# tonyckc/WT-PSE-code

Hardware: AMD Instinct MI355X
Metric: training images/sec (256x256 fundus) — full WT-PSE iteration (higher is better)
Workload: dtype f32 (layers with > 16 output channels and the fused 1x1 heads: x2h (2 fp16 terms per fp32 operand — power-of-two operand scaling —, 3 fp16 MFMA products per multiply, fp32 accumulation); the 16-channel layers the same on 16x16x32, the 1-/3-channel input layers and small 1x1 convs fp32-input MFMA)

## Files before the change

include/wtpse_hip.h:

```cpp
#ifndef WTPSE_HIP_H
#define WTPSE_HIP_H
#ifdef __cplusplus
extern "C" {
#endif


int wtpse_pack_conv_weights(const float* params, const int* desc, int n_desc, float* packed, void* stream);

int wtpse_conv_fwd(const float* in0, int C0, const float* in1, int C1, const float* wpacked, const float* bias,
                   const float* pro0, const float* pro1, int pro_relu, float* out0, float* out1, int Csplit, float* stats,
                   int B, int H, int W, int Cout, int ksize, int relu_out, const float* mask_ref, unsigned* out_amax, void* stream);
int wtpse_conv_stats_blocks(int B, int H, int W);
int wtpse_conv_fwd_gram(const float* in0, int C0, const float* wpacked, const float* bias, const float* pro0, int pro_relu,
                        float* out0, float* gram_partial, int B, int H, int W, int Cout, int relu_out, unsigned* out_amax,
                        void* stream);

int wtpse_conv_x3_stats_blocks(int B, int H, int W, int Cout, int ksize);
int wtpse_x3r_enable(int on);
int wtpse_x3_xcd(int on);
int wtpse_x3_small_wide(int on);
int wtpse_x3_terms(int terms);
int wtpse_amax(const float* x, long long n, unsigned* amax_table, void* stream);
int wtpse_pack_conv_weights_x3(const float* params, const int* desc, int n_desc, unsigned short* packed, void* stream);
int wtpse_conv_fwd_x3(const float* in0, int C0, const float* in1, int C1, const unsigned short* wpacked, const float* bias,
                      const float* pro0, const float* pro1, int pro_relu, float* out0, float* out1, int Csplit, float* stats,
                      int B, int H, int W, int Cout, int ksize, int relu_out, const float* mask_ref, const unsigned* in_amax,
                      const unsigned* in_amax1, unsigned* out_amax, void* stream);

int wtpse_conv16_x3(const float* in0, int C0, const unsigned short* wx16, const float* bias, const float* pro0, int pro_relu,
                    float* out0, float* stats, float* gram_partial, const float* mask_ref, const float* bn_ss,
                    const float* bn_mean, int bn_relu, int B, int H, int W, int Cout, int relu_out, int in_is_grad,
                    const unsigned* in_amax, unsigned* out_amax, void* stream);
int wtpse_pack_conv16_x3(const float* params, const int* desc, int n_desc, unsigned short* packed, void* stream);

int wtpse_dgrad_bnb(const float* dy, int C, const float* wpacked, float* out0, float* out1, int Csplit, const float* bn_y,
                    const float* bn_ss, const float* bn_mean, int bn_relu, int bn_c0, int bn_c1, float* stats, int B, int H, int W,
                    int Cout, int ksize, void* stream);
int wtpse_dgrad_x3_bnb(const float* dy, int C, const unsigned short* wpacked, float* out0, float* out1, int Csplit,
                       const float* bn_y, const float* bn_ss, const float* bn_mean, int bn_relu, int bn_c0, int bn_c1, float* stats,
                       int B, int H, int W, int Cout, int ksize, const unsigned* in_amax, void* stream);

int wtpse_conv_fwd_bnf(const float* in0, int C0, const float* in1, int C1, const void* wpacked, int layout, const float* bias,
                       const float* pro0, const float* pro1, int pro_relu, float* out0, float* stats, const float* gamma,
                       const float* beta, float* running_mean, float* running_var, long long* num_batches, float momentum, float eps,
                       float* scale_shift, float* save_mean, float* save_invstd, double* partial2, unsigned* tickets, int B, int H,
// ... 72 lines not shown
                                   int HW, unsigned* amax, void* stream);
int wtpse_bn_bwd_finalize_coef_frozen(const float* stats_partial, int nblk, int C, const float* gamma, const float* invstd,
                                      float* coef, float* dgamma, float* dbeta, float* dbias, int accumulate, void* stream);
int wtpse_bn_bwd_scale_coef(const float* g, const float* coef, float* dy, int B, int C, int HW, unsigned* amax, void* stream);

int wtpse_wt_loss_fwd(const float* z, int B, int C, int HW, float eps, float margin, int domain_num, int per_domain,
                      float* partial, float* gram, float* v, float* offdiag, float* diag, double* rowval,
                      float* dmmd_dv, float* losses, void* stream);
int wtpse_wt_split(int B, int HW, int* chunk_out);
int wtpse_wt_loss_fwd_partials(const float* partial, int S, int B, int HW, float eps, float margin, int domain_num,
                               int per_domain, float* gram, float* v, float* offdiag, float* diag, double* rowval,
                               float* dmmd_dv, float* losses, void* stream);
int wtpse_wt_gram_fwd(const float* z, int B, int C, int HW, float eps, float* partial, float* gram, float* v, float* offdiag,
                      float* diag, void* stream);
int wtpse_wt_final(const float* offdiag, const float* diag, int B, int Bnorm, float margin, const double* rowval, int R,
                   float* losses, void* stream);
int wtpse_wt_loss_bwd(const float* z, int B, int C, int HW, float margin, int domain_num, int per_domain,
                      const float* gram, const float* offdiag, const float* diag, const float* dmmd_dv,
                      const float* g_off, const float* g_diag, const float* g_dom, float w_off, float w_diag, float w_dom,
                      float* Mws, float* dz, int accumulate, void* stream);
int wtpse_wt_combine(const float* losses, int nmaps, float den, int mode, float* out, void* stream);
int wtpse_mmd_fwd(const float* v, int domain_num, int per_domain, double* rowval, float* dmmd_dv, void* stream);

int wtpse_maxpool2_fwd(const float* x, const float* pro, int relu, float* out, int B, int C, int H, int W, void* stream);
int wtpse_maxpool2_bwd(const float* x, const float* pro, int relu, const float* dout, float* dx, int accumulate, int B,
                       int C, int H, int W, void* stream);
int wtpse_maxpool2_bwd_stats_blocks(int B, int H, int W);
int wtpse_maxpool2_bwd_bnb(const float* x, const float* pro, int relu, const float* dout, float* dx, int accumulate,
                           const float* mean, float* stats, int B, int C, int H, int W, void* stream);
int wtpse_upsample2x_fwd(const float* x, const float* pro, int relu, float* out, int B, int C, int H, int W, void* stream);
int wtpse_upsample2x_bwd(const float* dout, float* dx, int accumulate, int B, int C, int H, int W, unsigned* amax, void* stream);
int wtpse_upsample2x_bwd_bn(const float* g, const float* bn_y, const float* bn_coef, float* dx, int B, int C, int H, int W,
                            unsigned* amax, void* stream);
int wtpse_upsample2x_fwd_stats(const float* x, float* out, float* stats, int B, int C, int H, int W, void* stream);
int wtpse_upsample2x_stats_blocks(int B, int H, int W);

int wtpse_resize_bilinear(const float* x, float* out, int B, int C, int H, int W, int Ho, int Wo, void* stream);

int wtpse_attn_fuse_fwd(const float* z, const float* wb, const float* emb, float coef, float* att, float* att_pre,
                        float* mask, float* fuse, int B, int CE, int HW, void* stream);
int wtpse_attn_fuse_bwd(const float* dfuse, const float* z, const float* emb, const float* att, const float* wb, float coef,
                        float* demb, float* dz, float* partial, float* d_wb, int accumulate, int B, int CE, int HW,
                        void* stream);

int wtpse_reparam_fwd(const float* mu, const float* logvar, const float* eps, float* z, long long n, void* stream);
int wtpse_reparam_bwd(const float* dz, const float* logvar, const float* eps, float* dlogvar, long long n, void* stream);
int wtpse_exp_half(const float* logvar, float* std_, long long n, void* stream);
int wtpse_reparam_student(const float* mu, const float* std_, const float* eps, float* z, long long n, void* stream);
int wtpse_nan_scrub(float* x, long long n, int* flag, void* stream);
int wtpse_randn(float* out, long long n, unsigned long long seed, unsigned long long offset,
                const unsigned long long* offset_dev, void* stream);
int wtpse_counter_add(void* counter, long long inc, int is64, void* stream);

int wtpse_reduce_blocks(long long n);
int wtpse_bce_sigmoid_fwd(const float* x, const float* t, long long n, float* partial, float* loss, void* stream);
int wtpse_bce_sigmoid_bwd(const float* x, const float* t, const float* g, float w, long long n, float* dx, void* stream);
int wtpse_pos_weight(const float* mask, const float* t, long long n, float* partial, float* sums, float* pw, void* stream);
int wtpse_pos_weight_from_sums(const float* sums, float* pw, void* stream);
int wtpse_bce_logits_pw_fwd(const float* x, const float* mask, const float* t, const float* pw, long long n, float* partial,
                            float* loss, void* stream);
int wtpse_bce_logits_pw_bwd(const float* x, const float* mask, const float* t, const float* pw, const float* g, float w,
                            long long n, float* dx, void* stream);
int wtpse_mse_fwd(const float* a, const float* b, long long n, float* partial, float* loss, void* stream);
int wtpse_mse_bwd(const float* a, const float* b, const float* g, float w, long long n, float* da, void* stream);
int wtpse_roi(const float* image, const float* logit, float* roi, float* od_pred, int B, int C, int HW, void* stream);
int wtpse_adam(float* p, const float* g, float* m, float* v, long long n, double lr, double beta1, double beta2, double eps,
// ... 118 lines not shown
```

wt-pse-code_amd/wtpse_hip/csrc/conv.hip:

```cpp
#include "internal.h"

#define WTPSE_P16_KC(KS) ((KS) == 3 ? 4 : 8)

struct ConvArgs {
  const float* in0;
  const float* in1;
  const float* wp;
  const float* bias;
  const float* pro0;
  const float* pro1;
  float* out0;
  float* out1;
  float* stats;
  const float* mask;
  const unsigned* in_amax;
  float in_scale;
  unsigned* out_amax;
  float* gram;
  const float* bn_ss;
  const float* bn_mean;
  int bn_c0, bn_c1, bn_relu;
  BnbTail tail;
  BnfTail ftail;
  int B, H, W;
  int C0, C1, Cin, CinP;
  int Cout, CoutP, Csplit;
  int pro_relu;
  int relu_out;
  int tiles_x, tiles_y;
  int xcd_tiles;
};


template <bool P16> struct AccT { typedef f32x16 type; };
template <> struct AccT<true> { typedef f32x4 type; };
__device__ __forceinline__ f32x4 mfma(float a, float b, f32x4 c) { return mfma16(a, b, c); }
__device__ __forceinline__ f32x16 mfma(float a, float b, f32x16 c) { return mfma32(a, b, c); }

template <int PE>
struct PlaneStride {
  static constexpr int value = ((PE - 16 + 31) / 32) * 32 + 16;
};

template <int KS, int MODE, int TWL, bool DB, int EPI>
__global__ __launch_bounds__(256, 3) void conv_fwd_k(ConvArgs a) {
  constexpr bool MASK = EPI == 1, BNB = EPI == 2;
  constexpr int TAPS = KS * KS, PAD = KS / 2;
  constexpr int TW = 1 << TWL, TH = 256 / TW;
  constexpr int PITCH = TW + 2 * PAD, ROWS = TH + 2 * PAD;
  constexpr int PE = PITCH * ROWS;
  constexpr int NPOS = (PE + 255) / 256;
  constexpr int S = PlaneStride<NPOS * 256>::value;
  constexpr bool XP = (MODE == 3 || MODE == 4);
  constexpr int XT = MODE == 4 ? 2 : 3;
  constexpr bool P16 = (MODE == 0) || XP;
  static_assert(!XP || KS == 3, "MODE 3 / 4 is the 3x3 path");
  constexpr int MT = P16 ? 1 : MODE;
  constexpr int MB = P16 ? 16 : 32;
  constexpr int CB = MB * MT;
  constexpr int NT = P16 ? 4 : 2;
  constexpr int NB = P16 ? 16 : 32;
  constexpr int KC = P16 ? WTPSE_P16_KC(KS) : 8;
  constexpr int KQ = P16 ? 4 : 2;
  constexpr int NACC = P16 ? 4 : 16;
  constexpr int CB4 = CB / 4;
  constexpr int NW = (KC * TAPS * CB4 + 255) / 256;
  constexpr int PEP = (PE + 7) & ~7;
  constexpr int XS_SZ = XP ? 2 * XT * PEP * 4 : KC * S;
  constexpr int WS_SZ = XP ? 0 : NW * 1024;
  constexpr int GRAM_SZ = (P16 && KS == 3) ? 4 * 16 * 65 + 4 * 256 : 0;
  constexpr int RED_SZ = 4 * CB * 2 > GRAM_SZ ? 4 * CB * 2 : GRAM_SZ;
  constexpr int MAIN_SZ = (XS_SZ + WS_SZ) > RED_SZ ? (XS_SZ + WS_SZ) : RED_SZ;
  __shared__ __attribute__((aligned(16))) float smem[MAIN_SZ + CB + (BNB ? 4 * CB : 0)];
  float* bias_s = smem + MAIN_SZ;
  const float* bnp_s = bias_s + CB;
  float* Xs = smem;
  float* Ws = smem + XS_SZ;

  const int tid = threadIdx.x, lane = tid & 63, wave = tid >> 6;
  int tile = (int)blockIdx.x, cblk = (int)blockIdx.y;
  if (a.xcd_tiles > 0) {
    const int L = (int)(blockIdx.y * gridDim.x + blockIdx.x), sl = L >> 3;
    cblk = sl % (int)gridDim.y;
    tile = (L & 7) * a.xcd_tiles + sl / (int)gridDim.y;
  }
  int bx = tile;
  const int tx = bx % a.tiles_x;
  bx /= a.tiles_x;
  const int ty = bx % a.tiles_y;
  const int b = bx / a.tiles_y;
  const int cout0 = cblk * CB;
  const int HW = a.H * a.W;
  if (tid < CB) bias_s[tid] = (a.bias && cout0 + tid < a.Cout) ? a.bias[cout0 + tid] : 0.f;
  if (BNB && tid < CB) bnb_stage<CB>(bias_s + CB + tid, cout0 + tid, a);

  int off[NT];
#pragma unroll
  for (int nt = 0; nt < NT; ++nt) {
    int p = wave * 64 + nt * NB + (lane & (NB - 1));
    off[nt] = (p >> TWL) * PITCH + (p & (TW - 1));
  }

  typename AccT<P16>::type acc[MT][NT];
// ... 90 lines not shown
      const int t = min(2 * s5 + (g4 >> 1), TAPS - 1);
      toff[s5] = (t / KS) * PITCH + (t % KS);
    }
    const int hsel = (g4 & 1) * PEP;
#pragma unroll
    for (int nt = 0; nt < NT; ++nt) {
#pragma unroll
      for (int s5 = 0; s5 < 5; ++s5) {
        u32x4 bfr[XT];
#pragma unroll
        for (int t = 0; t < XT; ++t) bfr[t] = Xq[(t * 2) * PEP + hsel + off[nt] + toff[s5]];
        f32x4 c = acc[0][nt];
        if constexpr (XT == 3) {
          c = wt_mfma16x32(afr[s5][0], bfr[2], c);
          c = wt_mfma16x32(afr[s5][1], bfr[1], c);
          c = wt_mfma16x32(afr[s5][2], bfr[0], c);
          c = wt_mfma16x32(afr[s5][0], bfr[1], c);
          c = wt_mfma16x32(afr[s5][1], bfr[0], c);
          c = wt_mfma16x32(afr[s5][0], bfr[0], c);
        } else {
          c = wt_mfma16x32h(afr[s5][0], bfr[1], c);
          c = wt_mfma16x32h(afr[s5][1], bfr[0], c);
          c = wt_mfma16x32h(afr[s5][0], bfr[0], c);
        }
        acc[0][nt] = c;
      }
    }
    if constexpr (MODE == 4) {
      const float inv = a.wp[0] / sx;
#pragma unroll
      for (int nt = 0; nt < NT; ++nt) acc[0][nt] *= inv;
    }
    __syncthreads();
  } else {
  int gpos[NPOS];
#pragma unroll
  for (int i = 0; i < NPOS; ++i) {
    int p = tid + 256 * i;
    int r = p / PITCH, x = p - r * PITCH;
    int gy = ty * TH + r - PAD, gx = tx * TW + x - PAD;
    gpos[i] = (p < PE && gy >= 0 && gy < a.H && gx >= 0 && gx < a.W) ? gy * a.W + gx : -1;
  }

  const __amdgpu_buffer_rsrc_t rs0 = make_rsrc(a.in0 + (size_t)b * a.C0 * HW, (unsigned)a.C0 * HW * 4u);
  const __amdgpu_buffer_rsrc_t rs1 = a.in1 ? make_rsrc(a.in1 + (size_t)b * a.C1 * HW, (unsigned)a.C1 * HW * 4u) : rs0;
  unsigned voff[NPOS];
#pragma unroll
  for (int i = 0; i < NPOS; ++i) voff[i] = gpos[i] >= 0 ? (unsigned)gpos[i] * 4u : BUF_OOB;
  const __amdgpu_buffer_rsrc_t rsw = make_rsrc(a.wp, (unsigned)a.CinP * TAPS * (unsigned)a.CoutP * 4u);
  unsigned woff[NW];
#pragma unroll
  for (int it = 0; it < NW; ++it) {
    const int e4 = tid + 256 * it;
    const int row = e4 / CB4, j4 = e4 - row * CB4;
    woff[it] = (row < KC * TAPS && cout0 + j4 * 4 < a.CoutP) ? (unsigned)(row * a.CoutP + cout0 + j4 * 4) * 4u : BUF_OOB;
  }
  const bool any_pro = a.pro0 != nullptr || a.pro1 != nullptr || a.pro_relu != 0;
  float xv[KC][NPOS];
  f32x4 wv[NW];
  auto issue_loads = [&](int c0) {
    const bool first = c0 < a.C0;
    const __amdgpu_buffer_rsrc_t rs = first ? rs0 : rs1;
    const int cbase = first ? c0 : c0 - a.C0;
    const int cmax = (first ? a.C0 : a.C1) - 1;
#pragma unroll
    for (int c = 0; c < KC; ++c) {
// ... 86 lines not shown
    int p = wave * 64 + nt * NB + (lane & (NB - 1));
    int gy = ty * TH + (p >> TWL), gx = tx * TW + (p & (TW - 1));
    poff[nt] = (gy < a.H && gx < a.W) ? gy * a.W + gx : -1;
  }
  const __amdgpu_buffer_rsrc_t rs_o0 = make_rsrc(a.out0 + (size_t)b * a.Csplit * HW, (unsigned)a.Csplit * HW * 4u);
  const __amdgpu_buffer_rsrc_t rs_o1 = a.out1 ? make_rsrc(a.out1 + (size_t)b * C1out * HW, (unsigned)C1out * HW * 4u) : rs_o0;
  const int Cbn = a.bn_c1 - a.bn_c0;
  const __amdgpu_buffer_rsrc_t rs_m = MASK ? make_rsrc(a.mask + (size_t)b * a.Cout * HW, (unsigned)a.Cout * HW * 4u)
                                      : BNB ? make_rsrc(a.mask + (size_t)b * Cbn * HW, (unsigned)Cbn * HW * 4u) : rs_o0;
  const int clane = P16 ? (lane >> 4) * 4 : (lane >> 5) * 4;
  unsigned pvo[NT];
#pragma unroll
  for (int nt = 0; nt < NT; ++nt) pvo[nt] = poff[nt] >= 0 ? (unsigned)(clane * HW + poff[nt]) * 4u : BUF_OOB;
  constexpr int NSV = NACC * 2;
  const bool full = ty * TH + TH <= a.H && tx * TW + TW <= a.W && cout0 + CB <= a.Cout;
  if (!full) {
#pragma unroll
    for (int mt = 0; mt < MT; ++mt)
#pragma unroll
      for (int r = 0; r < NACC; ++r) {
        const bool cvalid = cout0 + (P16 ? r : (mt * 32 + (r & 3) + 8 * (r >> 2))) + clane < a.Cout;
#pragma unroll
        for (int nt = 0; nt < NT; ++nt) acc[mt][nt][r] = (cvalid && poff[nt] >= 0) ? acc[mt][nt][r] : 0.f;
      }
  }
  if (a.relu_out) {
#pragma unroll
    for (int mt = 0; mt < MT; ++mt)
#pragma unroll
      for (int nt = 0; nt < NT; ++nt)
#pragma unroll
        for (int r = 0; r < NACC; ++r) acc[mt][nt][r] = out_clamp<EPI>(acc[mt][nt][r], 0.f);
  }
  if constexpr (P16 && KS == 3) {
    if (a.gram) {
      __syncthreads();
      float* zs = smem + wave * (16 * 65);
#pragma unroll
      for (int nt = 0; nt < NT; ++nt)
#pragma unroll
        for (int r = 0; r < NACC; ++r) zs[((lane >> 4) * 4 + r) * 65 + nt * 16 + (lane & 15)] = acc[0][nt][r];
      __builtin_amdgcn_wave_barrier();
      f32x4 g = {0.f, 0.f, 0.f, 0.f};
#pragma unroll
      for (int st = 0; st < 16; ++st) {
        const float v = zs[(lane & 15) * 65 + 4 * st + (lane >> 4)];
        g = mfma16(v, v, g);
      }
      float* gs = smem + 4 * 16 * 65 + wave * 256;
#pragma unroll
      for (int r = 0; r < 4; ++r) gs[((lane >> 4) * 4 + r) * 16 + (lane & 15)] = g[r];
      __syncthreads();
      const float* g0 = smem + 4 * 16 * 65;
      a.gram[(size_t)tile * 256 + tid] = g0[tid] + g0[256 + tid] + g0[512 + tid] + g0[768 + tid];
      __syncthreads();
    }
  }
  if constexpr (EPI == 0) {
    if (a.out_amax) {
      unsigned am = 0u;
#pragma unroll
      for (int mt = 0; mt < MT; ++mt)
#pragma unroll
        for (int nt = 0; nt < NT; ++nt)
#pragma unroll
          for (int r = 0; r < NACC; ++r) am = max(am, amax_bits(acc[mt][nt][r]));
      amax_publish_wave(a.out_amax, am, (unsigned)tile * 4u + (unsigned)wave);
// ... 107 lines not shown
      }
    }
  }
  TailTicket tk;
  tk.old = 0u;
  tk.armed = 0;
  if (defer) {
    if constexpr (BNB) tk = bnb_tail_begin<CB>(a.tail, a.bn_c0, a.bn_c1, cout0, tile, cblk, tid);
    else tk = bnf_tail_begin(a.ftail, tile, cblk, tid);
  }
  if (defer) {
#pragma unroll
    for (int mt = 0; mt < MT; ++mt)
#pragma unroll
      for (int r = 0; r < NACC; ++r) {
        const int cbase = cout0 + (P16 ? r : (mt * 32 + (r & 3) + 8 * (r >> 2)));
        const bool second = a.out1 != nullptr && cbase >= a.Csplit;
        const __amdgpu_buffer_rsrc_t rs_o = second ? rs_o1 : rs_o0;
        const unsigned soff = (unsigned)(second ? min(cbase, a.Cout) - a.Csplit : min(cbase, a.Csplit)) * hw4;
#pragma unroll
        for (int nt = 0; nt < NT; ++nt) buf_store(rs_o, pvo[nt], soff, acc[mt][nt][r]);
      }
    if constexpr (BNB)
      bnb_tail<CB>(tk, a.tail, a.stats, a.bn_mean, a.bn_c0, a.bn_c1, cout0, tile, cblk, tid,
                   reinterpret_cast<double*>(red), reinterpret_cast<int*>(red + 520));
    else
      bnf_tail<CB>(tk, a.ftail, a.stats, a.Cout, cout0, tile, cblk, tid, reinterpret_cast<double*>(red),
                   reinterpret_cast<int*>(red + 520));
  }
}

template <int KS, int MODE, bool DB, int EPI>
static int launch_fwd(const ConvArgs& a, hipStream_t st) {
  constexpr int CB = (MODE == 0 || MODE == 3 || MODE == 4) ? 16 : 32 * MODE;
  ConvArgs args = a;
  const Tiling t = conv_tiling(a.B, a.H, a.W);
  args.tiles_x = t.tiles_x;
  args.tiles_y = t.tiles_y;
  dim3 grid((unsigned)t.tiles, (unsigned)ceil_div(a.CoutP, CB));
  static const bool xcd_on = [] { const char* e = getenv("WTPSE_C16_XCD"); return !(e && e[0] == '0'); }();
  args.xcd_tiles = (xcd_on && grid.x % 8 == 0 && (long long)grid.x * grid.y >= 64) ? (int)(grid.x / 8) : 0;
  const bool in_launch = tail_in_launch((long long)grid.x * grid.y);
  if (!in_launch) args.tail.tickets = args.ftail.tickets = nullptr;
  if (args.tail.tickets) bnb_tail_geometry(args.tail, (int)grid.x, a.Cout, (double)a.B * a.H * a.W);
  if (args.ftail.tickets) bnf_tail_geometry(args.ftail, (int)grid.x, a.Cout, (double)a.B * a.H * a.W);
  if (t.TW == 16)
    hipLaunchKernelGGL((conv_fwd_k<KS, MODE, 4, DB, EPI>), grid, dim3(256), 0, st, args);
  else
    hipLaunchKernelGGL((conv_fwd_k<KS, MODE, 5, DB, EPI>), grid, dim3(256), 0, st, args);
  const int rc = wtpse_status();
  return rc == 0 && !in_launch ? tail_after_launch(a, (int)grid.x, st) : rc;
}

extern "C" int wtpse_conv_stats_blocks(int B, int H, int W) { return conv_tiling(B, H, W).tiles; }

static int conv_check(const ConvCall& c, int layout) {
  const BnbArgs& bn = c.bn;
  const BnbTail& t = c.tail;
  const BnfTail& f = c.ftail;
  const bool bnb = bn.mean != nullptr;
  WTPSE_REQUIRE(layout == CONV_FP32 || layout == CONV_X3 || layout == CONV_C16);
  WTPSE_REQUIRE(c.in0 && c.w && c.out0 && c.B > 0 && c.H > 0 && c.W > 0 && c.C0 > 0 && c.C1 >= 0 && c.Cout > 0);
  WTPSE_REQUIRE(c.ksize == 1 || c.ksize == 3);
  WTPSE_REQUIRE((c.C1 == 0) == (c.in1 == nullptr));
  WTPSE_REQUIRE(c.Csplit > 0 && c.Csplit <= c.Cout && ((c.Csplit == c.Cout) == (c.out1 == nullptr)));
  WTPSE_REQUIRE(c.Csplit == c.Cout || c.Csplit % 16 == 0);
  WTPSE_REQUIRE(!(c.stats && c.relu_out));
  WTPSE_REQUIRE(bnb || !(c.stats && c.mask_ref));
  WTPSE_REQUIRE(bnb || !(c.mask_ref && c.out1));
  WTPSE_REQUIRE(!bnb || (c.mask_ref && c.stats && bn.ss && !c.bias && !c.relu_out && !c.gram && bn.c0 >= 0 && bn.c0 < bn.c1 &&
                         bn.c1 <= c.Cout && bn.c0 % 16 == 0 && (bn.c1 % 16 == 0 || bn.c1 == c.Cout)));
  WTPSE_REQUIRE(c.C1 == 0 || c.C0 % 16 == 0);
  WTPSE_REQUIRE(!(c.out_amax && (c.mask_ref || bnb)));
  WTPSE_REQUIRE(!c.gram || (c.Cout == 16 && !c.relu_out));
  WTPSE_REQUIRE(!t.tickets || (bnb && t.partial2 && t.gamma && t.invstd && t.coef && t.dgamma && t.dbeta));
  WTPSE_REQUIRE(!f.tickets || (!bnb && c.stats && !c.gram && f.partial2 && f.gamma && f.beta && f.scale_shift && f.save_mean &&
                               f.save_invstd && (f.rmean == nullptr) == (f.rvar == nullptr)));
  if (layout == CONV_X3) {
    const X3Tiling g = x3_tiling(c.B, c.H, c.W, c.Cout, c.ksize);
    WTPSE_REQUIRE(!c.gram && !(c.in_amax1 && !c.in1) && ((c.C0 + c.C1 + 15) & ~15) <= (g.mt == 2 && !g.half ? 512 : 256));
  }
  if (layout == CONV_C16)
    WTPSE_REQUIRE(c.ksize == 3 && c.C0 <= 16 && c.Cout <= 16 && (((uintptr_t)c.w) & 15) == 0 && !c.in1 && !c.pro1);
  return 0;
}

static int conv_launch_fwd(const ConvCall& c, bool c16, hipStream_t st) {
  const bool bnb = c.bn.mean != nullptr;
  ConvArgs a;
  a.tail = c.tail;
  a.ftail = c.ftail;
  a.bn_ss = c.bn.ss; a.bn_mean = c.bn.mean; a.bn_relu = c.bn.relu; a.bn_c0 = bnb ? c.bn.c0 : 0; a.bn_c1 = bnb ? c.bn.c1 : 0;
  a.in0 = c.in0; a.in1 = c.in1; a.wp = static_cast<const float*>(c.w); a.bias = c.bias; a.pro0 = c.pro0; a.pro1 = c.pro1;
  a.out0 = c.out0; a.out1 = c.out1; a.stats = c.stats; a.mask = c.mask_ref; a.gram = c.gram;
  a.in_amax = c16 ? c.in_amax0 : nullptr; a.in_scale = c16 ? X3_FWD_SCALE : 1.f; a.out_amax = c.out_amax;
  a.B = c.B; a.H = c.H; a.W = c.W; a.C0 = c.C0; a.C1 = c.C1; a.Cin = c.C0 + c.C1; a.CinP = c16 ? 16 : (a.Cin + 3) & ~3;
  a.Cout = c.Cout; a.CoutP = (c.Cout + 15) & ~15; a.Csplit = c.Csplit; a.pro_relu = c.pro_relu; a.relu_out = c.relu_out;
  a.tiles_x = a.tiles_y = 0;
#define FWD(KS, M, DB) (bnb ? launch_fwd<KS, M, DB, 2>(a, st) : c.mask_ref ? launch_fwd<KS, M, DB, 1>(a, st) : launch_fwd<KS, M, DB, 0>(a, st))
  if (c16) return (g_x3_terms == 2 && (!c.in_is_grad || c.in_amax0)) ? FWD(3, 4, false) : FWD(3, 3, false);
  int mode = c.Cout <= 16 ? 0 : (c.Cout % 64 == 0 ? 2 : 1);
  const int tiles = conv_tiling(c.B, c.H, c.W).tiles;
  if (mode == 2 && tiles * (a.CoutP / 64) < 512) mode = 1;
  if (mode == 1 && tiles * ceil_div(a.CoutP, 32) < 384) mode = 0;
  const int cb = mode == 0 ? 16 : 32 * mode;
  const bool db = tiles * ceil_div(a.CoutP, cb) < 768 && a.CinP > (mode == 0 ? WTPSE_P16_KC(c.ksize) : 8);
#define FWD_DB(KS, M) (db ? FWD(KS, M, true) : FWD(KS, M, false))
  if (c.ksize == 3) return mode == 0 ? FWD_DB(3, 0) : mode == 1 ? FWD_DB(3, 1) : FWD_DB(3, 2);
  return mode == 0 ? FWD_DB(1, 0) : mode == 1 ? FWD_DB(1, 1) : FWD_DB(1, 2);
#undef FWD_DB
#undef FWD
}

int conv_run(const ConvCall& c, int layout, hipStream_t st) {
  if (const int rc = conv_check(c, layout)) return rc;
  return layout == CONV_X3 ? conv_launch_x3(c, st) : conv_launch_fwd(c, layout == CONV_C16, st);
}

extern "C" int wtpse_conv_fwd(const float* in0, int C0, const float* in1, int C1, const float* wpacked,
                              const float* bias, const float* pro0, const float* pro1, int pro_relu, float* out0, float* out1,
                              int Csplit, float* stats, int B, int H, int W, int Cout, int ksize, int relu_out,
                              const float* mask_ref, unsigned* out_amax, void* stream) {
  ConvCall c;
  c.in0 = in0; c.C0 = C0; c.in1 = in1; c.C1 = C1; c.w = wpacked; c.bias = bias; c.pro0 = pro0; c.pro1 = pro1; c.pro_relu = pro_relu;
  c.out0 = out0; c.out1 = out1; c.Csplit = Csplit; c.stats = stats; c.mask_ref = mask_ref; c.out_amax = out_amax;
  c.B = B; c.H = H; c.W = W; c.Cout = Cout; c.ksize = ksize; c.relu_out = relu_out;
  return conv_run(c, CONV_FP32, (hipStream_t)stream);
}

extern "C" int wtpse_dgrad_bnb(const float* dy, int C, const float* wpacked, float* out0, float* out1, int Csplit,
                               const float* bn_y, const float* bn_ss, const float* bn_mean, int bn_relu, int bn_c0, int bn_c1,
                               float* stats, int B, int H, int W, int Cout, int ksize, void* stream) {
  WTPSE_REQUIRE(bn_y && bn_ss && bn_mean && stats);
// ... 540 lines not shown
```

wt-pse-code_amd/wtpse_hip/csrc/pointwise.hip:

```cpp
#include "common.h"

__device__ __forceinline__ float act_in(float v, const float* pro, int c, int relu) {
  if (pro) v = fmaf(v, pro[2 * c], pro[2 * c + 1]);
  return relu ? fmaxf(v, 0.f) : v;
}

__device__ __forceinline__ float block_sum(float v, float* sh4) {
  v = wave_xor_sum(v, 32);
  __syncthreads();
  if ((threadIdx.x & 63) == 0) sh4[threadIdx.x >> 6] = v;
  __syncthreads();
  return sh4[0] + sh4[1] + sh4[2] + sh4[3];
}

__global__ __launch_bounds__(256) void maxpool2_fwd_k(const float* __restrict__ x, const float* __restrict__ pro, int relu,
                                                      float* __restrict__ out, int C, int H, int W, long long total) {
  const int Ho = H / 2, Wo = W / 2;
  long long i = (long long)blockIdx.x * 256 + threadIdx.x;
  if (i >= total) return;
  int xo = (int)(i % Wo);
  long long r = i / Wo;
  int yo = (int)(r % Ho);
  long long bc = r / Ho;
  int c = (int)(bc % C);
// ... 272 lines not shown
        const float* yrow = bn_y + (size_t)bc * Ho * Wo + (size_t)yo * Wo + 2 * xb;
        const float4 y0 = *reinterpret_cast<const float4*>(yrow), y1 = *reinterpret_cast<const float4*>(yrow + 4);
        const float v[10] = {xb > 0 ? yrow[-1] : 0.f, y0.x, y0.y, y0.z, y0.w, y1.x, y1.y, y1.z, y1.w, 2 * xb + 8 < Wo ? yrow[8] : 0.f};
#pragma unroll
        for (int t = 0; t < 10; ++t) w[t] = bn_dy(k1, k2, k3, w[t], v[t]);
        if (xb == 0) w[0] = 0.f;
        if (2 * xb + 8 >= Wo) w[9] = 0.f;
      }
#pragma unroll
      for (int e = 0; e < 4; ++e) {
        const int xx = xb + e;
        float rowsum = 0.f;
#pragma unroll
        for (int dxo = -1; dxo <= 2; ++dxo) {
          const int xo = 2 * xx + dxo;
          if (xo < 0 || xo >= Wo) continue;
          rowsum += up_w(xo, W, xx) * w[2 * e + dxo + 1];
        }
        g[e] += wy * rowsum;
      }
    }
    float* dst = dx + (size_t)bc * H * W + (size_t)yy * W + xb;
    float4 o = make_float4(g[0], g[1], g[2], g[3]);
    if (accumulate) {
      const float4 p = *reinterpret_cast<const float4*>(dst);
      o = make_float4(p.x + o.x, p.y + o.y, p.z + o.z, p.w + o.w);
    }
    *reinterpret_cast<float4*>(dst) = o;
    am = max(am, max(max(amax_bits(o.x), amax_bits(o.y)), max(amax_bits(o.z), amax_bits(o.w))));
  }
  if (amax) amax_publish_wave(amax, am, (blockIdx.x + blockIdx.y * gridDim.x) * 4u + (threadIdx.x >> 6));
}

__global__ __launch_bounds__(256) void resize_bilinear_k(const float* __restrict__ x, float* __restrict__ out, int H, int W,
                                                         int Ho, int Wo, float sy, float sx, long long total) {
  long long i = (long long)blockIdx.x * 256 + threadIdx.x;
  if (i >= total) return;
  int xo = (int)(i % Wo);
  long long r = i / Wo;
  int yo = (int)(r % Ho);
  long long bc = r / Ho;
  float fy = sy * (yo + 0.5f) - 0.5f, fx = sx * (xo + 0.5f) - 0.5f;
  if (fy < 0.f) fy = 0.f;
  if (fx < 0.f) fx = 0.f;
  int y0 = (int)fy, x0 = (int)fx;
  int y1 = y0 + (y0 < H - 1 ? 1 : 0), x1 = x0 + (x0 < W - 1 ? 1 : 0);
  float ly = fy - (float)y0, lx = fx - (float)x0;
  const float* src = x + (size_t)bc * H * W;
  float v00 = src[y0 * W + x0], v01 = src[y0 * W + x1], v10 = src[y1 * W + x0], v11 = src[y1 * W + x1];
  out[i] = (1.f - ly) * ((1.f - lx) * v00 + lx * v01) + ly * ((1.f - lx) * v10 + lx * v11);
}

__global__ __launch_bounds__(256) void relu_mask_k(const float* __restrict__ dz, const float* __restrict__ ref,
                                                   float* __restrict__ dy, int accumulate, long long n) {
  long long i = (long long)blockIdx.x * 256 + threadIdx.x;
  if (i >= n) return;
  float g = ref[i] > 0.f ? dz[i] : 0.f;
  dy[i] = accumulate ? dy[i] + g : g;
}

__global__ __launch_bounds__(256) void axpy_k(float* __restrict__ dst, const float* __restrict__ src, float alpha, long long n) {
  long long i = (long long)blockIdx.x * 256 + threadIdx.x;
  if (i < n) dst[i] = fmaf(alpha, src[i], dst[i]);
}

__global__ __launch_bounds__(256) void relu_mask_v_k(const float4* __restrict__ dz, const float4* __restrict__ ref,
// ... 330 lines not shown
  if (W % 4 == 0 && H % 2 == 0 && (((uintptr_t)x | (uintptr_t)dx | (uintptr_t)dout) & 15) == 0)
    hipLaunchKernelGGL(maxpool2_bwd_v_k, PLANE_GRID((H / 2) * (W / 4), B * C), dim3(256), 0, ST, x, pro, relu, dout, dx, accumulate,
                       B * C, C, H, W, (const float*)nullptr, (float*)nullptr);
  else
    hipLaunchKernelGGL(maxpool2_bwd_k, GRID1(total), dim3(256), 0, ST, x, pro, relu, dout, dx, accumulate, C, H, W, total);
  return wtpse_status();
}
extern "C" int wtpse_maxpool2_bwd_stats_blocks(int B, int H, int W) { return B * (((H / 2) * (W / 4) + 255) / 256); }
extern "C" int wtpse_maxpool2_bwd_bnb(const float* x, const float* pro, int relu, const float* dout, float* dx, int accumulate,
                                      const float* mean, float* stats, int B, int C, int H, int W, void* stream) {
  WTPSE_REQUIRE(x && pro && dout && dx && mean && stats && B > 0 && C > 0 && H >= 2 && W >= 4);
  WTPSE_REQUIRE(W % 4 == 0 && H % 2 == 0 && (((uintptr_t)x | (uintptr_t)dx | (uintptr_t)dout) & 15) == 0);
  WTPSE_REQUIRE(B * C < 32768);
  hipLaunchKernelGGL(maxpool2_bwd_v_k, PLANE_GRID((H / 2) * (W / 4), B * C), dim3(256), 0, ST, x, pro, relu, dout, dx,
                     (accumulate & 1) | 2, B * C, C, H, W, mean, stats);
  return wtpse_status();
}
extern "C" int wtpse_upsample2x_fwd(const float* x, const float* pro, int relu, float* out, int B, int C, int H, int W, void* stream) {
  WTPSE_REQUIRE(x && out && B > 0 && C > 0 && H > 0 && W > 0);
  long long total = (long long)B * C * H * W * 4;
  if (W % 2 == 0 && W >= 2 && (((uintptr_t)out) & 15) == 0)
    hipLaunchKernelGGL(upsample2x_fwd4_v_k, PLANE_GRID((H + 1) * (W / 2), B * C), dim3(256), 0, ST, x, pro, relu, out, nullptr, B * C, C, H, W);
  else
    hipLaunchKernelGGL(upsample2x_fwd_k, GRID1(total), dim3(256), 0, ST, x, pro, relu, out, C, H, W, total);
  return wtpse_status();
}
extern "C" int wtpse_upsample2x_stats_blocks(int B, int H, int W) { return B * (((H + 1) * (W / 2) + 255) / 256); }
extern "C" int wtpse_upsample2x_fwd_stats(const float* x, float* out, float* stats, int B, int C, int H, int W, void* stream) {
  WTPSE_REQUIRE(x && out && stats && B > 0 && C > 0 && H > 0 && W >= 2 && W % 2 == 0 && (((uintptr_t)out) & 15) == 0);
  WTPSE_REQUIRE(B * C < 32768);
  hipLaunchKernelGGL(upsample2x_fwd4_v_k, PLANE_GRID((H + 1) * (W / 2), B * C), dim3(256), 0, ST, x, nullptr, 0, out, stats, B * C, C, H, W);
  return wtpse_status();
}
static inline dim3 up_bwd_grid(int per_plane, int planes, bool) { return PLANE_GRID(per_plane, planes); }
extern "C" int wtpse_upsample2x_bwd(const float* dout, float* dx, int accumulate, int B, int C, int H, int W, unsigned* amax, void* stream) {
  WTPSE_REQUIRE(dout && dx && B > 0 && C > 0 && H > 0 && W > 0);
  long long total = (long long)B * C * H * W;
  if (W % 4 == 0 && (((uintptr_t)dout | (uintptr_t)dx) & 15) == 0) {
    hipLaunchKernelGGL(upsample2x_bwd_v_k<false>, up_bwd_grid(H * (W / 4), B * C, amax != nullptr), dim3(256), 0, ST, dout, dx, accumulate,
                       B * C, H, W, nullptr, nullptr, C, amax);
    return wtpse_status();
  }
  hipLaunchKernelGGL(upsample2x_bwd_k, GRID1(total), dim3(256), 0, ST, dout, dx, accumulate, H, W, total);
  const int rc = wtpse_status();
  return (rc || !amax) ? rc : wtpse_amax(dx, total, amax, stream);
}
extern "C" int wtpse_upsample2x_bwd_bn(const float* g, const float* bn_y, const float* bn_coef, float* dx, int B, int C, int H, int W,
                                       unsigned* amax, void* stream) {
  WTPSE_REQUIRE(g && bn_y && bn_coef && dx && B > 0 && C > 0 && H > 0 && W > 0 && W % 4 == 0);
  WTPSE_REQUIRE((((uintptr_t)g | (uintptr_t)bn_y | (uintptr_t)dx) & 15) == 0);
  hipLaunchKernelGGL(upsample2x_bwd_v_k<true>, up_bwd_grid(H * (W / 4), B * C, amax != nullptr), dim3(256), 0, ST, g, dx, 0, B * C, H, W,
                     bn_y, bn_coef, C, amax);
  return wtpse_status();
}
extern "C" int wtpse_resize_bilinear(const float* x, float* out, int B, int C, int H, int W, int Ho, int Wo, void* stream) {
  WTPSE_REQUIRE(x && out && B > 0 && C > 0 && H > 0 && W > 0 && Ho > 0 && Wo > 0);
  long long total = (long long)B * C * Ho * Wo;
  hipLaunchKernelGGL(resize_bilinear_k, GRID1(total), dim3(256), 0, ST, x, out, H, W, Ho, Wo, (float)H / (float)Ho,
                     (float)W / (float)Wo, total);
  return wtpse_status();
}
extern "C" int wtpse_relu_mask(const float* dz, const float* ref, float* dy, int accumulate, long long n, void* stream) {
  WTPSE_REQUIRE(dz && ref && dy && n > 0);
  if (n % 4 == 0 && (((uintptr_t)dz | (uintptr_t)ref | (uintptr_t)dy) & 15) == 0)
    hipLaunchKernelGGL(relu_mask_v_k, GRID1(n / 4), dim3(256), 0, ST, reinterpret_cast<const float4*>(dz),
                       reinterpret_cast<const float4*>(ref), reinterpret_cast<float4*>(dy), accumulate, n / 4);
  else
    hipLaunchKernelGGL(relu_mask_k, GRID1(n), dim3(256), 0, ST, dz, ref, dy, accumulate, n);
  return wtpse_status();
}
__global__ __launch_bounds__(256) void copy_w16_k(const float4* __restrict__ src, float4* __restrict__ dst, long long n4) {
  for (long long i = (long long)blockIdx.x * 256 + threadIdx.x; i < n4; i += (long long)gridDim.x * 256) dst[i] = src[i];
}
__global__ __launch_bounds__(256) void copy_w4_k(const float* __restrict__ src, float* __restrict__ dst, long long n) {
  for (long long i = (long long)blockIdx.x * 256 + threadIdx.x; i < n; i += (long long)gridDim.x * 256) dst[i] = src[i];
}
extern "C" int wtpse_copy_probe(const float* src, float* dst, long long n, int bytes_per_lane, void* stream) {
  WTPSE_REQUIRE(src && dst && n > 0 && n % 4 == 0 && (bytes_per_lane == 4 || bytes_per_lane == 16));
  WTPSE_REQUIRE((((uintptr_t)src | (uintptr_t)dst) & 15) == 0);
  if (bytes_per_lane == 16)
    hipLaunchKernelGGL(copy_w16_k, dim3(8192), dim3(256), 0, ST, reinterpret_cast<const float4*>(src), reinterpret_cast<float4*>(dst), n / 4);
  else
    hipLaunchKernelGGL(copy_w4_k, dim3(16384), dim3(256), 0, ST, src, dst, n);
  return wtpse_status();
}
// ... 200 lines not shown
```

Before: 816.3.

## Add specialized first-layer 3x3 conv path and LDS-staged upsample backward kernel

Adds a MODE 5 forward conv path for 3x3 layers with at most 4 input channels and 16 outputs. It keeps the weights in registers, uses one 16x16x4 MFMA k-step per tap, drops weight LDS staging and allows higher occupancy (launch bound 6). It also adds an upsample-2x backward kernel that stages the needed output-gradient rows in LDS before the bilinear adjoint, so each dout value is read once per block instead of reloaded per output. The new paths add code and LDS use, and the upsample kernel's row mapping and grid-stride loop over planes are more complex.

```diff
diff --git a/include/wtpse_hip.h b/include/wtpse_hip.h
--- a/include/wtpse_hip.h
+++ b/include/wtpse_hip.h
@@ -11,6 +11,8 @@
                    const float* pro0, const float* pro1, int pro_relu, float* out0, float* out1, int Csplit, float* stats,
                    int B, int H, int W, int Cout, int ksize, int relu_out, const float* mask_ref, unsigned* out_amax, void* stream);
 int wtpse_conv_stats_blocks(int B, int H, int W);
+int wtpse_first_conv(int on);
+int wtpse_first_conv_takes(int ksize, int C0, int C1, int Cout, int mask, int bnb, int gram);
 int wtpse_conv_fwd_gram(const float* in0, int C0, const float* wpacked, const float* bias, const float* pro0, int pro_relu,
                         float* out0, float* gram_partial, int B, int H, int W, int Cout, int relu_out, unsigned* out_amax,
                         void* stream);
@@ -149,6 +151,7 @@
 int wtpse_upsample2x_bwd(const float* dout, float* dx, int accumulate, int B, int C, int H, int W, unsigned* amax, void* stream);
 int wtpse_upsample2x_bwd_bn(const float* g, const float* bn_y, const float* bn_coef, float* dx, int B, int C, int H, int W,
                             unsigned* amax, void* stream);
+int wtpse_up_bwd_planes(int planes);
 int wtpse_upsample2x_fwd_stats(const float* x, float* out, float* stats, int B, int C, int H, int W, void* stream);
 int wtpse_upsample2x_stats_blocks(int B, int H, int W);
 
diff --git a/wt-pse-code_amd/wtpse_hip/csrc/conv.hip b/wt-pse-code_amd/wtpse_hip/csrc/conv.hip
--- a/wt-pse-code_amd/wtpse_hip/csrc/conv.hip
+++ b/wt-pse-code_amd/wtpse_hip/csrc/conv.hip
@@ -43,8 +43,10 @@
 };
 
 template <int KS, int MODE, int TWL, bool DB, int EPI>
-__global__ __launch_bounds__(256, 3) void conv_fwd_k(ConvArgs a) {
+__global__ __launch_bounds__(256, MODE == 5 ? 6 : 3) void conv_fwd_k(ConvArgs a) {
   constexpr bool MASK = EPI == 1, BNB = EPI == 2;
+  constexpr bool FIRST = MODE == 5;
+  static_assert(!FIRST || (KS == 3 && EPI == 0 && !DB), "MODE 5 is the plain 3x3 forward of the first layers");
   constexpr int TAPS = KS * KS, PAD = KS / 2;
   constexpr int TW = 1 << TWL, TH = 256 / TW;
   constexpr int PITCH = TW + 2 * PAD, ROWS = TH + 2 * PAD;
@@ -53,7 +55,7 @@
   constexpr int S = PlaneStride<NPOS * 256>::value;
   constexpr bool XP = (MODE == 3 || MODE == 4);
   constexpr int XT = MODE == 4 ? 2 : 3;
-  constexpr bool P16 = (MODE == 0) || XP;
+  constexpr bool P16 = (MODE == 0) || XP || FIRST;
   static_assert(!XP || KS == 3, "MODE 3 / 4 is the 3x3 path");
   constexpr int MT = P16 ? 1 : MODE;
   constexpr int MB = P16 ? 16 : 32;
@@ -67,8 +69,9 @@
   constexpr int NW = (KC * TAPS * CB4 + 255) / 256;
   constexpr int PEP = (PE + 7) & ~7;
   constexpr int XS_SZ = XP ? 2 * XT * PEP * 4 : KC * S;
-  constexpr int WS_SZ = XP ? 0 : NW * 1024;
-  constexpr int GRAM_SZ = (P16 && KS == 3) ? 4 * 16 * 65 + 4 * 256 : 0;
+  constexpr int WS_SZ = (XP || FIRST) ? 0 : NW * 1024;
+  constexpr int GRAM_SZ = (P16 && KS == 3 && !FIRST) ? 4 * 16 * 65 + 4 * 256 : 0;
+  static_assert(!FIRST || XS_SZ >= 524, "the statistics tail takes 256 doubles and a flag of this LDS");
   constexpr int RED_SZ = 4 * CB * 2 > GRAM_SZ ? 4 * CB * 2 : GRAM_SZ;
   constexpr int MAIN_SZ = (XS_SZ + WS_SZ) > RED_SZ ? (XS_SZ + WS_SZ) : RED_SZ;
   __shared__ __attribute__((aligned(16))) float smem[MAIN_SZ + CB + (BNB ? 4 * CB : 0)];
@@ -225,6 +228,54 @@
       for (int nt = 0; nt < NT; ++nt) acc[0][nt] *= inv;
     }
     __syncthreads();
+  } else if constexpr (FIRST) {
+    static_assert(KC == 4 && KQ == 4, "one 16x16x4 k-step");
+    const int cl = lane >> 4;
+    float av[TAPS];
+#pragma unroll
+    for (int t = 0; t < TAPS; ++t) av[t] = a.wp[(cl * TAPS + t) * CB + (lane & 15)];
+    const __amdgpu_buffer_rsrc_t rs0 = make_rsrc(a.in0 + (size_t)b * a.C0 * HW, (unsigned)a.C0 * HW * 4u);
+    bool in_img[NPOS];
+    float xv[KC][NPOS];
+#pragma unroll
+    for (int i = 0; i < NPOS; ++i) {
+      const int p = tid + 256 * i;
+      const int r = p / PITCH, x = p - r * PITCH;
+      const int gy = ty * TH + r - PAD, gx = tx * TW + x - PAD;
+      in_img[i] = p < PE && gy >= 0 && gy < a.H && gx >= 0 && gx < a.W;
+      const unsigned vo = in_img[i] ? (unsigned)(gy * a.W + gx) * 4u : BUF_OOB;
+#pragma unroll
+      for (int c = 0; c < KC; ++c) xv[c][i] = buf_load(rs0, vo, (unsigned)min(c, a.C0 - 1) * (unsigned)HW * 4u);
+    }
+    if (a.pro0 != nullptr || a.pro_relu != 0) {
+      const bool relu = a.pro_relu & 1;
+#pragma unroll
+      for (int c = 0; c < KC; ++c) {
+        const int cg = min(c, a.C0 - 1);
+        const float sc = a.pro0 ? a.pro0[2 * cg] : 1.f, sh = a.pro0 ? a.pro0[2 * cg + 1] : 0.f;
+#pragma unroll
+        for (int i = 0; i < NPOS; ++i) {
+          float v = fmaf(xv[c][i], sc, sh);
+          if (relu) v = fmaxf(v, 0.f);
+          xv[c][i] = in_img[i] ? v : 0.f;
+        }
+      }
+    }
+#pragma unroll
+    for (int c = 0; c < KC; ++c)
+#pragma unroll
+      for (int i = 0; i < NPOS; ++i) Xs[c * S + tid + 256 * i] = xv[c][i];
+    __syncthreads();
+    const float* xrow = Xs + cl * S;
+    float bv[TAPS][NT];
+#pragma unroll
+    for (int t = 0; t < TAPS; ++t)
+#pragma unroll
+      for (int nt = 0; nt < NT; ++nt) bv[t][nt] = xrow[off[nt] + (t / KS) * PITCH + (t % KS)];
+#pragma unroll
+    for (int t = 0; t < TAPS; ++t)
+#pragma unroll
+      for (int nt = 0; nt < NT; ++nt) acc[0][nt] = mfma(av[t], bv[t][nt], acc[0][nt]);
   } else {
   int gpos[NPOS];
 #pragma unroll
@@ -377,7 +428,7 @@
 #pragma unroll
         for (int r = 0; r < NACC; ++r) acc[mt][nt][r] = out_clamp<EPI>(acc[mt][nt][r], 0.f);
   }
-  if constexpr (P16 && KS == 3) {
+  if constexpr (P16 && KS == 3 && !FIRST) {
     if (a.gram) {
       __syncthreads();
       float* zs = smem + wave * (16 * 65);
@@ -551,7 +602,7 @@
 
 template <int KS, int MODE, bool DB, int EPI>
 static int launch_fwd(const ConvArgs& a, hipStream_t st) {
-  constexpr int CB = (MODE == 0 || MODE == 3 || MODE == 4) ? 16 : 32 * MODE;
+  constexpr int CB = (MODE == 0 || MODE >= 3) ? 16 : 32 * MODE;
   ConvArgs args = a;
   const Tiling t = conv_tiling(a.B, a.H, a.W);
   args.tiles_x = t.tiles_x;
@@ -604,6 +655,19 @@
   return 0;
 }
 
+static int g_first_conv = [] { const char* e = getenv("WTPSE_FIRST_CONV"); return !(e && e[0] == '0') ? 1 : 0; }();
+extern "C" int wtpse_first_conv(int on) {
+  const int was = g_first_conv;
+  if (on == 0 || on == 1) g_first_conv = on;
+  return was;
+}
+static bool conv_first_takes(int ksize, int C0, bool second_input, int Cout, bool mask, bool bnb, bool gram) {
+  return g_first_conv && ksize == 3 && !second_input && C0 <= 4 && Cout <= 16 && !mask && !bnb && !gram;
+}
+extern "C" int wtpse_first_conv_takes(int ksize, int C0, int C1, int Cout, int mask, int bnb, int gram) {
+  return conv_first_takes(ksize, C0, C1 > 0, Cout, mask != 0, bnb != 0, gram != 0) ? 1 : 0;
+}
+
 static int conv_launch_fwd(const ConvCall& c, bool c16, hipStream_t st) {
   const bool bnb = c.bn.mean != nullptr;
   ConvArgs a;
@@ -618,6 +682,8 @@
   a.tiles_x = a.tiles_y = 0;
 #define FWD(KS, M, DB) (bnb ? launch_fwd<KS, M, DB, 2>(a, st) : c.mask_ref ? launch_fwd<KS, M, DB, 1>(a, st) : launch_fwd<KS, M, DB, 0>(a, st))
   if (c16) return (g_x3_terms == 2 && (!c.in_is_grad || c.in_amax0)) ? FWD(3, 4, false) : FWD(3, 3, false);
+  if (conv_first_takes(c.ksize, c.C0, c.in1 != nullptr || c.pro1 != nullptr, c.Cout, c.mask_ref != nullptr, bnb, c.gram != nullptr))
+    return launch_fwd<3, 5, false, 0>(a, st);
   int mode = c.Cout <= 16 ? 0 : (c.Cout % 64 == 0 ? 2 : 1);
   const int tiles = conv_tiling(c.B, c.H, c.W).tiles;
   if (mode == 2 && tiles * (a.CoutP / 64) < 512) mode = 1;
diff --git a/wt-pse-code_amd/wtpse_hip/csrc/pointwise.hip b/wt-pse-code_amd/wtpse_hip/csrc/pointwise.hip
--- a/wt-pse-code_amd/wtpse_hip/csrc/pointwise.hip
+++ b/wt-pse-code_amd/wtpse_hip/csrc/pointwise.hip
@@ -328,6 +328,87 @@
   if (amax) amax_publish_wave(amax, am, (blockIdx.x + blockIdx.y * gridDim.x) * 4u + (threadIdx.x >> 6));
 }
 
+template <bool BN>
+__global__ __launch_bounds__(256) void upsample2x_bwd_s_k(const float* __restrict__ dout, float* __restrict__ dx, int accumulate,
+                                                          int BC, int H, int W, const float* __restrict__ bn_y,
+                                                          const float* __restrict__ bn_coef, int C, unsigned* __restrict__ amax) {
+  extern __shared__ __attribute__((aligned(16))) float up_rows[];
+  const int Ho = 2 * H, Wo = 2 * W, W4 = W / 4;
+  const int Q = 2 * W4, P = Wo + 8;
+  const int tid = threadIdx.x, j0 = blockIdx.x * 256, j = j0 + tid;
+  const bool live = j < H * W4;
+  const int k = j % W4, yy = j / W4;
+  const int xb = 4 * k;
+  const int yyA = j0 / W4, yyB = min(j0 + 255, H * W4 - 1) / W4;
+  const int ybase = 2 * yyA - 1;
+  const int total = (2 * (yyB - yyA + 1) + 2) * Q;
+  const int dq = 256 / Q, dr = 256 % Q;
+  const int s0 = tid / Q, c40 = tid - s0 * Q;
+  const bool x_first = xb == 0, x_last = xb + 4 == W;
+  const float wx[4][4] = {{x_first ? 0.f : 0.25f, x_first ? 1.f : 0.75f, 0.75f, 0.25f}, {0.25f, 0.75f, 0.75f, 0.25f},
+                          {0.25f, 0.75f, 0.75f, 0.25f}, {0.25f, 0.75f, x_last ? 1.f : 0.75f, x_last ? 0.f : 0.25f}};
+  const float wy[4] = {0.25f, yy == 0 ? 1.f : 0.75f, yy == H - 1 ? 1.f : 0.75f, 0.25f};
+  unsigned am = 0u;
+  for (int bc = blockIdx.y; bc < BC; bc += gridDim.y) {
+    const float* src = dout + (size_t)bc * Ho * Wo;
+    const float* ysrc = BN ? bn_y + (size_t)bc * Ho * Wo : nullptr;
+    float k1 = 1.f, k2 = 0.f, k3 = 0.f;
+    if (BN) {
+      const int c = bc % C;
+      k1 = bn_coef[3 * c]; k2 = bn_coef[3 * c + 1]; k3 = bn_coef[3 * c + 2];
+    }
+    int s = s0, c4 = c40;
+    for (int base = 0; base < total; base += 1024) {
+      float4 gq[4], yq[4];
+      int lo[4];
+#pragma unroll
+      for (int u = 0; u < 4; ++u) {
+        lo[u] = base + u * 256 + tid < total ? s * P + 4 + 4 * c4 : -1;
+        const unsigned go = (unsigned)(min(max(ybase + s, 0), Ho - 1) * Wo + 4 * c4);
+        gq[u] = *reinterpret_cast<const float4*>(src + go);
+        if (BN) yq[u] = *reinterpret_cast<const float4*>(ysrc + go);
+        c4 += dr; s += dq;
+        if (c4 >= Q) { c4 -= Q; ++s; }
+      }
+#pragma unroll
+      for (int u = 0; u < 4; ++u)
+        if (lo[u] >= 0) *reinterpret_cast<float4*>(up_rows + lo[u]) = BN ? bn_dy4(k1, k2, k3, gq[u], yq[u]) : gq[u];
+    }
+    __syncthreads();
+    if (live) {
+      float g[4] = {0.f, 0.f, 0.f, 0.f};
+#pragma unroll
+      for (int dy = -1; dy <= 2; ++dy) {
+        const int yo = 2 * yy + dy;
+        if (yo < 0 || yo >= Ho) continue;
+        const float* row = up_rows + (yo - ybase) * P + 4 + 2 * xb;
+        const float4 q0 = *reinterpret_cast<const float4*>(row), q1 = *reinterpret_cast<const float4*>(row + 4);
+        float w[10];
+        w[0] = xb > 0 ? row[-1] : 0.f;
+        w[1] = q0.x; w[2] = q0.y; w[3] = q0.z; w[4] = q0.w; w[5] = q1.x; w[6] = q1.y; w[7] = q1.z; w[8] = q1.w;
+        w[9] = 2 * xb + 8 < Wo ? row[8] : 0.f;
+#pragma unroll
+        for (int e = 0; e < 4; ++e) {
+          float rowsum = 0.f;
+#pragma unroll
+          for (int t = 0; t < 4; ++t) rowsum = fmaf(wx[e][t], w[2 * e + t], rowsum);
+          g[e] = fmaf(wy[dy + 1], rowsum, g[e]);
+        }
+      }
+      float* dst = dx + (size_t)bc * H * W + (size_t)yy * W + xb;
+      float4 o = make_float4(g[0], g[1], g[2], g[3]);
+      if (accumulate) {
+        const float4 p = *reinterpret_cast<const float4*>(dst);
+        o = make_float4(p.x + o.x, p.y + o.y, p.z + o.z, p.w + o.w);
+      }
+      *reinterpret_cast<float4*>(dst) = o;
+      am = max(am, max(max(amax_bits(o.x), amax_bits(o.y)), max(amax_bits(o.z), amax_bits(o.w))));
+    }
+    __syncthreads();
+  }
+  if (amax) amax_publish_wave(amax, am, (blockIdx.x + blockIdx.y * gridDim.x) * 4u + (threadIdx.x >> 6));
+}
+
 __global__ __launch_bounds__(256) void resize_bilinear_k(const float* __restrict__ x, float* __restrict__ out, int H, int W,
                                                          int Ho, int Wo, float sy, float sx, long long total) {
   long long i = (long long)blockIdx.x * 256 + threadIdx.x;
@@ -724,13 +805,39 @@
   hipLaunchKernelGGL(upsample2x_fwd4_v_k, PLANE_GRID((H + 1) * (W / 2), B * C), dim3(256), 0, ST, x, nullptr, 0, out, stats, B * C, C, H, W);
   return wtpse_status();
 }
-static inline dim3 up_bwd_grid(int per_plane, int planes, bool) { return PLANE_GRID(per_plane, planes); }
+static int g_up_bwd_planes = 32768;
+extern "C" int wtpse_up_bwd_planes(int planes) {
+  const int was = g_up_bwd_planes;
+  if (planes > 0) g_up_bwd_planes = planes < 32768 ? planes : 32768;
+  return was;
+}
+static inline dim3 up_bwd_grid(int per_plane, int planes) {
+  return dim3((unsigned)((per_plane + 255) / 256), (unsigned)(planes < g_up_bwd_planes ? planes : g_up_bwd_planes));
+}
+static inline unsigned up_bwd_rows_bytes(int H, int W) {
+  const int W4 = W / 4;
+  if (W4 > 256) return 0u;
+  int rows = 256 % W4 == 0 ? 256 / W4 : 255 / W4 + 2;
+  if (rows > H) rows = H;
+  const long long bytes = (long long)(2 * rows + 2) * (2 * W + 8) * 4;
+  return bytes <= 40960 ? (unsigned)bytes : 0u;
+}
+template <bool BN>
+static void up_bwd_launch(const float* dout, float* dx, int accumulate, int BC, int H, int W, const float* bn_y, const float* bn_coef,
+                          int C, unsigned* amax, hipStream_t st) {
+  const unsigned lds = up_bwd_rows_bytes(H, W);
+  if (lds)
+    hipLaunchKernelGGL(upsample2x_bwd_s_k<BN>, up_bwd_grid(H * (W / 4), BC), dim3(256), lds, st, dout, dx, accumulate, BC, H, W, bn_y,
+                       bn_coef, C, amax);
+  else
+    hipLaunchKernelGGL(upsample2x_bwd_v_k<BN>, up_bwd_grid(H * (W / 4), BC), dim3(256), 0, st, dout, dx, accumulate, BC, H, W, bn_y,
+                       bn_coef, C, amax);
+}
 extern "C" int wtpse_upsample2x_bwd(const float* dout, float* dx, int accumulate, int B, int C, int H, int W, unsigned* amax, void* stream) {
   WTPSE_REQUIRE(dout && dx && B > 0 && C > 0 && H > 0 && W > 0);
   long long total = (long long)B * C * H * W;
   if (W % 4 == 0 && (((uintptr_t)dout | (uintptr_t)dx) & 15) == 0) {
-    hipLaunchKernelGGL(upsample2x_bwd_v_k<false>, up_bwd_grid(H * (W / 4), B * C, amax != nullptr), dim3(256), 0, ST, dout, dx, accumulate,
-                       B * C, H, W, nullptr, nullptr, C, amax);
+    up_bwd_launch<false>(dout, dx, accumulate, B * C, H, W, nullptr, nullptr, C, amax, ST);
     return wtpse_status();
   }
   hipLaunchKernelGGL(upsample2x_bwd_k, GRID1(total), dim3(256), 0, ST, dout, dx, accumulate, H, W, total);
@@ -741,8 +848,7 @@
                                        unsigned* amax, void* stream) {
   WTPSE_REQUIRE(g && bn_y && bn_coef && dx && B > 0 && C > 0 && H > 0 && W > 0 && W % 4 == 0);
   WTPSE_REQUIRE((((uintptr_t)g | (uintptr_t)bn_y | (uintptr_t)dx) & 15) == 0);
-  hipLaunchKernelGGL(upsample2x_bwd_v_k<true>, up_bwd_grid(H * (W / 4), B * C, amax != nullptr), dim3(256), 0, ST, g, dx, 0, B * C, H, W,
-                     bn_y, bn_coef, C, amax);
+  up_bwd_launch<true>(g, dx, 0, B * C, H, W, bn_y, bn_coef, C, amax, ST);
   return wtpse_status();
 }
 extern "C" int wtpse_resize_bilinear(const float* x, float* out, int B, int C, int H, int W, int Ho, int Wo, void* stream) {
```

Result: no change. 822.0 (median of 6 runs) (+0.7%).
